# liudabao001/JABD-Joint-Attention-Based-Detector-for-small-face-detection

Hardware: AMD Instinct MI355X
Metric: images/sec at 1024x1024 bs32 (1/2/4/8 GPU); boxes/sec NMS (higher is better)
Workload: dtype fp32; 1 GPU; C2: JABD-MobileNetV3 RetinaFace (nets/retinaface_r.py) eval forward, weights_init weights; global_batch=32, image_size=1024, parallelism=replicas x1

## Files before the change

jabd-joint-attention-based-detector-for-small-face-detection_amd/csrc/expdw.hip:

```cpp
#include "expdw_shared.h"

namespace jabd {

template <int K, int S, int TH, int TW, int EC, bool SKIP, int NW, int SKC>
constexpr int xd1_min_wg() {
  using C = XdCfg<K, S, TH, TW, EC>;
  constexpr int bytes = C::LDS * 4 + K * K * (EC / 4) * 16 + (SKIP ? 10 * (SKC / 4) * 16 : 16);
  return (SKIP && NW == 4 && 4 * bytes <= 160 * 1024) ? 4 : 2;
}

template <int K, int S, int TH, int TW, int EC, int ACT, int KP, bool SKIP = false, int NW = 4,
          int SKC = 160, int KCC = 0, bool PRE = false>
__global__ __launch_bounds__(64 * NW, (xd1_min_wg<K, S, TH, TW, EC, SKIP, NW, SKC>())) void expdw1_kernel(const jabd_expdw_args p, const XdDivs dv,
                                                       int nitems) {
  static_assert(!PRE || (KCC == 1 && KP == 1), "PRE: one input stage");
  const int Kc = KCC ? KCC : p.Kc;
  using C = XdCfg<K, S, TH, TW, EC>;
  constexpr int T = 64 * NW;
  constexpr int NPF = (C::IPAD * 4 + T - 1) / T;
  constexpr int BPW = (C::NBLK + NW - 1) / NW;
  static_assert(NW % C::NNT == 0, "waves split evenly over the 16-channel tiles");
  constexpr int NWD = K * K * C::NC4;
  __shared__ __attribute__((aligned(16))) float lds[C::LDS];
  __shared__ float4 wsh[K * K][C::NC4];
  __shared__ float4 sws[SKIP ? 10 : 1][SKIP ? SKC / 4 : 1];
  XdItem it;
  XD_RT(0);
  XD_T(1);
  if (!xd_item<K, S, TH, TW, EC>(p, blockIdx.x, dv, nitems, it)) return;
  const bool skip = SKIP && it.c0 == 0;
  if (skip) {
    const int c4 = threadIdx.x & 63;
    if (c4 < (p.Cin >> 2))
      for (int q = threadIdx.x >> 6; q < 10; q += NW)
        sws[q][c4] = *reinterpret_cast<const float4*>((q < 9 ? p.sw + q * p.Cin : p.sb) + 4 * c4);
  }
  const bool interior =
      it.ih0 >= 0 && it.iw0 >= 0 && it.ih0 + C::IH <= p.H && it.iw0 + C::IW <= p.W;
  const int t = threadIdx.x, lane = t & 63, wave = t >> 6, j = lane & 15, g = lane >> 4;
  const int ntw = wave % C::NNT;
  const int nt = it.c0 / 16 + ntw;
  const bool ntv = nt < p.Ntiles;
  const int ntc = ntv ? nt : 0;
  const f32x4* wpk = reinterpret_cast<const f32x4*>(p.we);
  const int chb = it.c0 + 16 * ntw + 4 * g;
  const bool chok = chb < p.E;
  float4 pbi = *reinterpret_cast<const float4*>(p.be + (chok ? chb : 0));
  if (!chok) pbi = make_float4(0.f, 0.f, 0.f, 0.f);
  float4 pwd = make_float4(0.f, 0.f, 0.f, 0.f);
  if (t < NWD) {
    const int tp = t / C::NC4, cc = it.c0 + 4 * (t - tp * C::NC4);
    const float4 w = *reinterpret_cast<const float4*>(p.wd + tp * p.E + (cc < p.E ? cc : 0));
    pwd = cc < p.E ? w : make_float4(0.f, 0.f, 0.f, 0.f);
  }
  int c4, sl;
  dw_lane<C::NC4>(lane, c4, sl);
  const int chl = 4 * c4;
  const bool chv = it.c0 + chl < p.E;
  const float4 bias2 = *reinterpret_cast<const float4*>(p.bd + (chv ? it.c0 + chl : 0));
  f32x4 apre = (f32x4){0.f, 0.f, 0.f, 0.f};
  float4 bpre = make_float4(0.f, 0.f, 0.f, 0.f);
  if constexpr (PRE) {
    const f32x4 w = reinterpret_cast<const f32x4*>(p.pw)[lane];
    const float4 gt = *reinterpret_cast<const float4*>(p.pg + (int64_t)it.b * p.pg_bs + 4 * g);
    apre = (f32x4){w.x * gt.x, w.y * gt.y, w.z * gt.z, w.w * gt.w};
    bpre = *reinterpret_cast<const float4*>(p.pb + 4 * g);
  }
  const __amdgpu_buffer_rsrc_t xr = __builtin_amdgcn_make_buffer_rsrc(
      const_cast<float*>(p.x), (short)0, (int)(uint32_t)((int64_t)p.B * p.x_bs * 4), 0x00020000);
  const int cq = ((t >> 4) & 3) * 4;
  const int spx0 = (t >> 6) * 16 + (t & 15);
  float4 pf[KP][NPF];
  auto load_stage = [&](int kc, float4 (&dst)[NPF]) {
    const int cofs = 16 * kc + cq;
    const uint32_t base = (uint32_t)(it.b * p.x_bs + cofs);
    const bool cok = cofs < p.Cin;
#pragma unroll
    for (int u = 0; u < NPF; ++u) {
      const int px = u * 16 * NW + spx0;
      const int r = px / C::IW, c = px - r * C::IW;
      const int ih = it.ih0 + r, iw = it.iw0 + c;
      const bool ok = px < C::IPX && cok &&
                      (interior || ((unsigned)ih < (unsigned)p.H && (unsigned)iw < (unsigned)p.W));
      const uint32_t off = ok ? (base + (uint32_t)((ih * p.W + iw) * p.x_ps)) * 4u : 0xFFFFFFF0u;
      if (XD_SKIP & 16) dst[u] = make_float4(0.f, 0.f, 0.f, (float)off);
      else dst[u] = __builtin_bit_cast(float4, __builtin_amdgcn_raw_buffer_load_b128(xr, off, 0, 0));
    }
  };
  f32x4 acc[BPW];
  const f32x4 bias4 = (f32x4){pbi.x, pbi.y, pbi.z, pbi.w};
#pragma unroll
  for (int u = 0; u < BPW; ++u) acc[u] = bias4;
#pragma unroll
  for (int s = 0; s < KP; ++s)
    if (s < Kc) load_stage(s, pf[s]);
  const bool tail8 = KCC == 2 && (p.Cin & 15) == 8;
  for (int kc0 = 0; kc0 < Kc; kc0 += KP) {
#pragma unroll
    for (int s = 0; s < KP; ++s) {
      const int kc = kc0 + s;
      if (kc >= Kc) break;
      const bool tl = tail8 && kc == Kc - 1;
      f32x4 a;
      if (tl) {
        const float* wf = reinterpret_cast<const float*>(p.we) +
                          ((int64_t)(kc * p.Ntiles + ntc) * 64 + j) * 4 + g;
        a = (f32x4){wf[0], wf[64], 0.f, 0.f};
      } else {
        a = wpk[(kc * p.Ntiles + ntc) * 64 + lane];
      }
#pragma unroll
      for (int u = 0; u < NPF; ++u) {
        if (u * 16 * NW + spx0 < C::IPAD)
          *reinterpret_cast<float4*>(lds + (cq / 4 * C::IPAD + u * 16 * NW + spx0) * 4) = pf[s][u];
      }
      if (!ntv) a = (f32x4){0.f, 0.f, 0.f, 0.f};
      asm volatile("" : "+v"(a));
      lds_barrier();
      if (kc == 0) XD_T(2);
      if constexpr (PRE) {
        constexpr int BPP = (C::NPB + NW - 1) / NW;
        const __amdgpu_buffer_rsrc_t rr = __builtin_amdgcn_make_buffer_rsrc(
            const_cast<float*>(p.pres), (short)0, (int)(uint32_t)((int64_t)p.B * p.x_bs * 4),
            0x00020000);
        f32x4 pacc[BPP];
        float4 res[BPP];
        bool pin[BPP];
#pragma unroll
        for (int u = 0; u < BPP; ++u) {
          const int pb = wave + NW * u;
          const int px = pb * 16 + j;
          const int r = px / C::IW, c = px - r * C::IW;
          const int ih = it.ih0 + r, iw = it.iw0 + c;
          pin[u] = pb < C::NPB && px < C::IPX &&
                   (interior || ((unsigned)ih < (unsigned)p.H && (unsigned)iw < (unsigned)p.W));
          const uint32_t off =
              pin[u] ? (uint32_t)(it.b * p.x_bs + (ih * p.W + iw) * p.x_ps + 4 * g) * 4u : 0xFFFFFFF0u;
          res[u] = __builtin_bit_cast(float4, __builtin_amdgcn_raw_buffer_load_b128(rr, off, 0, 0));
          pacc[u] = (f32x4){bpre.x, bpre.y, bpre.z, bpre.w};
          if (pb < C::NPB) {
            const f32x4 bv = *reinterpret_cast<const f32x4*>(lds + (g * C::IPAD + px) * 4);
            pacc[u] = __builtin_amdgcn_mfma_f32_16x16x4f32(apre.x, bv.x, pacc[u], 0, 0, 0);
            pacc[u] = __builtin_amdgcn_mfma_f32_16x16x4f32(apre.y, bv.y, pacc[u], 0, 0, 0);
            pacc[u] = __builtin_amdgcn_mfma_f32_16x16x4f32(apre.z, bv.z, pacc[u], 0, 0, 0);
            pacc[u] = __builtin_amdgcn_mfma_f32_16x16x4f32(apre.w, bv.w, pacc[u], 0, 0, 0);
          }
        }
        lds_barrier();
#pragma unroll
        for (int u = 0; u < BPP; ++u) {
          const int pb = wave + NW * u;
          if (pb >= C::NPB) continue;
          float4 v = make_float4(pacc[u][0] + res[u].x, pacc[u][1] + res[u].y,
                                 pacc[u][2] + res[u].z, pacc[u][3] + res[u].w);
          if (p.pact == ACT_RELU) v = xd_act4<ACT_RELU>(v);
          else if (p.pact == ACT_HSWISH) v = xd_act4<ACT_HSWISH>(v);
          if (!pin[u]) v = make_float4(0.f, 0.f, 0.f, 0.f);
          *reinterpret_cast<float4*>(lds + (g * C::IPAD + pb * 16 + j) * 4) = v;
        }
        lds_barrier();
      }
      if (kc + KP < Kc) load_stage(kc + KP, pf[s]);
      const int sc = 16 * kc + 4 * (t >> 6);
      if (skip && wave < 4 && sc < p.Cin) {
        const int op = t & 63, orow = op / TW, ocol = op - orow * TW;
        const int oh = it.oh0 + orow, ow = it.ow0 + ocol;
        if (orow < TH && oh < p.OH && ow < p.OW) {
          const int sq = sc >> 2;
          float4 v = sws[9][sq];
          const float* xq = lds + ((t >> 6) * C::IPAD) * 4;
#pragma unroll 1
          for (int kh = 0; kh < 3; ++kh)
#pragma unroll
            for (int kw = 0; kw < 3; ++kw) {
              const int px = (2 * orow + kh + C::PAD - 1) * C::IW + 2 * ocol + kw + C::PAD - 1;
              const float4 xv = *reinterpret_cast<const float4*>(xq + px * 4);
              const float4 wv = sws[kh * 3 + kw][sq];
              v = fma4pk(xv, wv, v);
            }
          *reinterpret_cast<float4*>(p.sy + (int64_t)it.b * p.sy_bs +
                                     ((int64_t)oh * p.OW + ow) * p.sy_ps + sc) = v;
        }
      }
      if (ntv && !(XD_SKIP & 1) && tl) {
#pragma unroll
        for (int u = 0; u < BPW; ++u) {
          const int blk = wave + NW * u;
          if (blk < C::NBLK) {
            const int pb = blk / C::NNT;
            const float b0 = lds[(pb * 16 + j) * 4 + g];
            const float b1 = lds[(C::IPAD + pb * 16 + j) * 4 + g];
            acc[u] = __builtin_amdgcn_mfma_f32_16x16x4f32(a.x, b0, acc[u], 0, 0, 0);
            acc[u] = __builtin_amdgcn_mfma_f32_16x16x4f32(a.y, b1, acc[u], 0, 0, 0);
          }
        }
      } else if (ntv && !(XD_SKIP & 1)) {
#pragma unroll
        for (int u = 0; u < BPW; ++u) {
          const int blk = wave + NW * u;
          if (blk < C::NBLK) {
            const int pb = blk / C::NNT;
            const f32x4 bv = *reinterpret_cast<const f32x4*>(lds + (g * C::IPAD + pb * 16 + j) * 4);
            acc[u] = __builtin_amdgcn_mfma_f32_16x16x4f32(a.x, bv.x, acc[u], 0, 0, 0);
            acc[u] = __builtin_amdgcn_mfma_f32_16x16x4f32(a.y, bv.y, acc[u], 0, 0, 0);
            acc[u] = __builtin_amdgcn_mfma_f32_16x16x4f32(a.z, bv.z, acc[u], 0, 0, 0);
            acc[u] = __builtin_amdgcn_mfma_f32_16x16x4f32(a.w, bv.w, acc[u], 0, 0, 0);
          }
        }
      }
      lds_barrier();
    }
  }
  XD_T(3);
  if (XD_SKIP & 2) {
  } else if (interior) {
#pragma unroll
    for (int u = 0; u < BPW; ++u) {
      const int blk = wave + NW * u;
      if (blk < C::NBLK) {
        const int pb = blk / C::NNT;
        const int px = pb * 16 + j, q = 4 * ntw + g;
        const float4 o = xd_act4<ACT>(make_float4(acc[u][0], acc[u][1], acc[u][2], acc[u][3]));
        if (pb * 16 + 16 <= C::IPX || px < C::IPX)
          *reinterpret_cast<float4*>(lds + (q * C::QP + px) * 4) = o;
      }
    }
  } else {
#pragma unroll
    for (int u = 0; u < BPW; ++u) {
      const int blk = wave + NW * u;
      if (blk < C::NBLK) {
        const int pb = blk / C::NNT;
        const int px = pb * 16 + j, q = 4 * ntw + g;
        const int r = px / C::IW, c = px - r * C::IW;
        const int ih = it.ih0 + r, iw = it.iw0 + c;
        const bool ok = (unsigned)ih < (unsigned)p.H && (unsigned)iw < (unsigned)p.W;
        float4 o = xd_act4<ACT>(make_float4(acc[u][0], acc[u][1], acc[u][2], acc[u][3]));
        if (!ok) o = make_float4(0.f, 0.f, 0.f, 0.f);
        if (px < C::IPX) *reinterpret_cast<float4*>(lds + (q * C::QP + px) * 4) = o;
      }
    }
  }
  if (t < NWD) wsh[t / C::NC4][t % C::NC4] = pwd;
  __syncthreads();
  XD_T(4);

  constexpr int SPW = 64 / C::NC4;
  float4 psum = make_float4(0.f, 0.f, 0.f, 0.f);
  if (chv && !(XD_SKIP & 4)) {
    float* yb = p.y + (int64_t)it.b * p.y_bs + it.c0 + chl;
#pragma unroll 1
    for (int pass = 0; pass * T < C::ITEMS; ++pass) {
      const int strip = (pass * NW + wave) * SPW + sl;
      if (strip >= TH * C::NSTRIP) break;
      const int orow = strip / C::NSTRIP, st = strip - orow * C::NSTRIP;
      const int oh = it.oh0 + orow, owb = it.ow0 + st * C::PW;
      if (oh >= p.OH || owb >= p.OW) continue;
      float4 a2[C::PW];
#pragma unroll
      for (int o = 0; o < C::PW; ++o) a2[o] = bias2;
#pragma unroll 1
      for (int kh = 0; kh < K; ++kh) {
        const float* rowp = lds + (c4 * C::QP + (orow * S + kh) * C::IW + st * C::PW * S) * 4;
        float4 row[C::SPAN];
#pragma unroll
        for (int c = 0; c < C::SPAN; ++c)
          row[c] = *reinterpret_cast<const float4*>(rowp + c * 4);
        float4 wk[K];
#pragma unroll
        for (int kw = 0; kw < K; ++kw) wk[kw] = wsh[kh * K + kw][c4];
#pragma unroll
        for (int o = 0; o < C::PW; ++o)
#pragma unroll
          for (int kw = 0; kw < K; ++kw) {
            const float4 xv = row[o * S + kw], wv = wk[kw];
            a2[o] = fma4pk(xv, wv, a2[o]);
          }
      }
#pragma unroll
      for (int o = 0; o < C::PW; ++o) {
        if (owb + o >= p.OW) break;
        const float4 v = xd_act4<ACT>(a2[o]);
        *reinterpret_cast<float4*>(yb + ((int64_t)oh * p.OW + owb + o) * p.y_ps) = v;
        psum.x += v.x; psum.y += v.y; psum.z += v.z; psum.w += v.w;
      }
    }
  }
  XD_T(5);
  if (p.part && !(XD_SKIP & 8)) {
    constexpr int NX = C::NC4 == 16 ? 2 : C::NC4 == 8 ? 3 : 4;
    constexpr int X8[3] = {12, 20, 32}, X4[4] = {4, 8, 16, 32}, X16[2] = {16, 32};
#pragma unroll
    for (int r = 0; r < NX; ++r) {
      const int off = C::NC4 == 16 ? X16[r] : C::NC4 == 8 ? X8[r] : X4[r];
      psum.x += __shfl_xor(psum.x, off);
      psum.y += __shfl_xor(psum.y, off);
      psum.z += __shfl_xor(psum.z, off);
      psum.w += __shfl_xor(psum.w, off);
    }
    __syncthreads();
    float4* red = reinterpret_cast<float4*>(lds);
    if (lane < C::NC4) red[wave * C::NC4 + lane] = psum;
    __syncthreads();
    if (t < C::NC4 && it.c0 + 4 * t < p.E) {
      float4 v[NW];
#pragma unroll
      for (int w = 0; w < NW; ++w) v[w] = red[w * C::NC4 + t];
#pragma unroll
      for (int h = NW / 2; h >= 1; h >>= 1)
#pragma unroll
        for (int w = 0; w < h; ++w) {
          v[w].x += v[w + h].x;
          v[w].y += v[w + h].y;
          v[w].z += v[w + h].z;
          v[w].w += v[w + h].w;
        }
      const float4 sm = v[0];
      *reinterpret_cast<float4*>(p.part + ((int64_t)it.b * (int)dv.tiles_img.d + it.t_in) * p.E +
                                 it.c0 + 4 * t) = sm;
    }
  }
  XD_T(6);
  XD_RT(7);
}


template <int K, int EC, int NB, int R>
struct XsCfg {
  static constexpr int PAD = K / 2;
  static constexpr int NPX = 16 * NB, OWS = NPX - 2 * PAD;
  static constexpr int NR = R + 2 * PAD;
  static constexpr int EP = EC + 4;
  static constexpr int NT = EC / 16, NC4 = EC / 4;
  static constexpr int SPX = R * NPX;
  static constexpr int NPF = SPX * 4 / 256;
  static constexpr int NBLK = R * NB * NT, BPW = NBLK / 4;
  static constexpr int PW = 2, NSTRIP = OWS / PW;
  static constexpr int ITEMS = R * NSTRIP * NC4;
  static constexpr int SPAN = PW + K - 1;
  static constexpr int LDS_X = 16 * SPX, LDS_E = NR * NPX * EP;
  static_assert(SPX * 4 % 256 == 0 && NBLK % 4 == 0 && 4 % NT == 0, "strip shape");
  static_assert(OWS % PW == 0, "strip width");
  static_assert((LDS_X + LDS_E) * 4 + (K * K + 1) * EC * 4 <= 80 * 1024, "LDS");
  static_assert(LDS_X >= 4 * 256, "ECA reduction buffer aliases the stage buffer");
};

template <int K, int EC, int NB, int R, int ACT>
__global__ __launch_bounds__(256, 2) void expdw_strip_kernel(const jabd_expdw_args p,
                                                             const XdDivs dv, int nitems,
                                                             int nstrip, int hb) {
  using C = XsCfg<K, EC, NB, R>;
  __shared__ __attribute__((aligned(16))) float xs[C::LDS_X];
  __shared__ __attribute__((aligned(16))) float er[C::LDS_E];
  __shared__ float4 wsh[K * K + 1][C::NC4];
  float4* red = reinterpret_cast<float4*>(xs);
  const int i = blockIdx.x;
  if (i >= nitems) return;
  const int xcd = i & 7, q = i >> 3;
  const int qn = fdiv(q, dv.nch);
  const int chunk = q - qn * (int)dv.nch.d;
  const int tile = qn * 8 + xcd;
  if (tile >= p.B * (int)dv.tiles_img.d) return;
  const int b = fdiv(tile, dv.tiles_img);
  const int t_in = tile - b * (int)dv.tiles_img.d;
  const int band = t_in / nstrip, strip = t_in - band * nstrip;
  const int hb0 = band * hb, hb1 = min(hb0 + hb, p.OH);
  const int ow0 = strip * C::OWS, iw0 = ow0 - C::PAD;
  const int c0 = chunk * EC;
  const int t = threadIdx.x, lane = t & 63, j = lane & 15, g = lane >> 4;
  const int wave = t >> 6;
  const int ntw = wave % C::NT;
  const int nt = c0 / 16 + ntw;
  const bool ntv = nt < p.Ntiles;
  const int ntc = ntv ? nt : 0;
  const f32x4* wpk = reinterpret_cast<const f32x4*>(p.we);
  const int chb = c0 + 16 * ntw + 4 * g;
  const bool chok = chb < p.E;
  const float4 pbi = *reinterpret_cast<const float4*>(p.be + (chok ? chb : 0));
  const f32x4 bias4 = (f32x4){pbi.x, pbi.y, pbi.z, pbi.w};
  for (int u = t; u < (K * K + 1) * C::NC4; u += 256) {
    const int tp = u / C::NC4, cc = c0 + 4 * (u - tp * C::NC4);
    const float4 w = *reinterpret_cast<const float4*>((tp < K * K ? p.wd + tp * p.E : p.bd) +
                                                      (cc < p.E ? cc : 0));
    wsh[tp][u - tp * C::NC4] = cc < p.E ? w : make_float4(0.f, 0.f, 0.f, 0.f);
  }
  const __amdgpu_buffer_rsrc_t xr = __builtin_amdgcn_make_buffer_rsrc(
      const_cast<float*>(p.x), (short)0, (int)(uint32_t)((int64_t)p.B * p.x_bs * 4), 0x00020000);
  const int cq = ((t >> 4) & 3) * 4;
  const int spx0 = (t >> 6) * 16 + (t & 15);
  const int e0 = hb0 - C::PAD;
  const int nsteps = (hb1 - hb0 + 2 * C::PAD + R - 1) / R;
  const int nitem = nsteps * p.Kc;
  float4 pf[C::NPF];
  auto load_stage = [&](int it) {
    const int s = it / p.Kc, kc = it - s * p.Kc;
    const int cofs = 16 * kc + cq;
    const uint32_t base = (uint32_t)(b * p.x_bs + cofs);
    const bool cok = cofs < p.Cin;
#pragma unroll
    for (int u = 0; u < C::NPF; ++u) {
      const int px = u * 64 + spx0;
      const int r = px / C::NPX, c = px - r * C::NPX;
      const int ih = e0 + s * R + r, iw = iw0 + c;
      const bool ok = cok && (unsigned)ih < (unsigned)p.H && (unsigned)iw < (unsigned)p.W;
      const uint32_t off = ok ? (base + (uint32_t)((ih * p.W + iw) * p.x_ps)) * 4u : 0xFFFFFFF0u;
      pf[u] = __builtin_bit_cast(float4, __builtin_amdgcn_raw_buffer_load_b128(xr, off, 0, 0));
    }
  };
  int c4, sl;
  dw_lane<C::NC4>(lane, c4, sl);
  const int chl = 4 * c4;
  const bool chv = c0 + chl < p.E;
  float* yb = p.y + (int64_t)b * p.y_bs + c0 + chl;
  float4 psum = make_float4(0.f, 0.f, 0.f, 0.f);
  f32x4 acc[C::BPW];
  load_stage(0);
  for (int it = 0; it < nitem; ++it) {
    const int s = it / p.Kc, kc = it - s * p.Kc;
    if (kc == 0) {
#pragma unroll
      for (int u = 0; u < C::BPW; ++u) acc[u] = bias4;
    }
    f32x4 a = wpk[(kc * p.Ntiles + ntc) * 64 + lane];
#pragma unroll
    for (int u = 0; u < C::NPF; ++u)
      *reinterpret_cast<float4*>(xs + ((cq / 4) * C::SPX + u * 64 + spx0) * 4) = pf[u];
    if (!ntv) a = (f32x4){0.f, 0.f, 0.f, 0.f};
    asm volatile("" : "+v"(a));
    lds_barrier();
    if (it + 1 < nitem) load_stage(it + 1);
    if (ntv) {
#pragma unroll
      for (int u = 0; u < C::BPW; ++u) {
        const int pb = (wave + 4 * u) / C::NT;
        const f32x4 bv = *reinterpret_cast<const f32x4*>(xs + (g * C::SPX + pb * 16 + j) * 4);
        acc[u] = __builtin_amdgcn_mfma_f32_16x16x4f32(a.x, bv.x, acc[u], 0, 0, 0);
        acc[u] = __builtin_amdgcn_mfma_f32_16x16x4f32(a.y, bv.y, acc[u], 0, 0, 0);
        acc[u] = __builtin_amdgcn_mfma_f32_16x16x4f32(a.z, bv.z, acc[u], 0, 0, 0);
        acc[u] = __builtin_amdgcn_mfma_f32_16x16x4f32(a.w, bv.w, acc[u], 0, 0, 0);
      }
    }
    if (kc + 1 < p.Kc) {
      lds_barrier();
      continue;
    }
#pragma unroll
    for (int u = 0; u < C::BPW; ++u) {
      const int pb = (wave + 4 * u) / C::NT;
      const int px = pb * 16 + j;
      const int r = px / C::NPX, c = px - r * C::NPX;
      const int ih = e0 + s * R + r, iw = iw0 + c;
      const bool ok = chok && (unsigned)ih < (unsigned)p.H && (unsigned)iw < (unsigned)p.W;
      const int slot = (s * R + r) % C::NR;
      float4 o;
      o.x = ok ? xd_act<ACT>(acc[u][0]) : 0.f;
      o.y = ok ? xd_act<ACT>(acc[u][1]) : 0.f;
      o.z = ok ? xd_act<ACT>(acc[u][2]) : 0.f;
      o.w = ok ? xd_act<ACT>(acc[u][3]) : 0.f;
      *reinterpret_cast<float4*>(er + (slot * C::NPX + c) * C::EP + 16 * ntw + 4 * g) = o;
    }
    lds_barrier();
    if (chv) {
      const float4 bias2 = wsh[K * K][c4];
#pragma unroll 1
      for (int pass = 0; pass * 256 < C::ITEMS; ++pass) {
        const int item = (pass * 4 + wave) * (64 / C::NC4) + sl;
        if (item >= R * C::NSTRIP) break;
        const int orow = item / C::NSTRIP, st = item - orow * C::NSTRIP;
        const int oh = hb0 + s * R - 2 * C::PAD + orow;
        const int owb = ow0 + st * C::PW;
        if (oh < hb0 || oh >= hb1 || owb >= p.OW) continue;
        float4 a2[C::PW];
#pragma unroll
        for (int o = 0; o < C::PW; ++o) a2[o] = bias2;
#pragma unroll 1
        for (int kh = 0; kh < K; ++kh) {
          const int slot = (oh - e0 - C::PAD + kh) % C::NR;
          const float* rowp = er + (slot * C::NPX + st * C::PW) * C::EP + chl;
          float4 row[C::SPAN];
#pragma unroll
          for (int c = 0; c < C::SPAN; ++c)
            row[c] = *reinterpret_cast<const float4*>(rowp + c * C::EP);
          float4 wk[K];
#pragma unroll
          for (int kw = 0; kw < K; ++kw) wk[kw] = wsh[kh * K + kw][c4];
#pragma unroll
          for (int o = 0; o < C::PW; ++o)
#pragma unroll
            for (int kw = 0; kw < K; ++kw) {
              const float4 xv = row[o + kw], wv = wk[kw];
              a2[o] = fma4pk(xv, wv, a2[o]);
            }
        }
#pragma unroll
        for (int o = 0; o < C::PW; ++o) {
          if (owb + o >= p.OW) break;
          float4 v;
          v.x = xd_act<ACT>(a2[o].x);
          v.y = xd_act<ACT>(a2[o].y);
          v.z = xd_act<ACT>(a2[o].z);
          v.w = xd_act<ACT>(a2[o].w);
          *reinterpret_cast<float4*>(yb + ((int64_t)oh * p.OW + owb + o) * p.y_ps) = v;
          psum.x += v.x; psum.y += v.y; psum.z += v.z; psum.w += v.w;
        }
      }
    }
    lds_barrier();
  }
  if (p.part) {
    __syncthreads();
    red[t] = psum;
    __syncthreads();
    if (t < C::NC4 && c0 + 4 * t < p.E) {
      float4 sm = make_float4(0.f, 0.f, 0.f, 0.f);
      for (int u = 0; u < 256; ++u) {
        int cu, su;
        dw_lane<C::NC4>(u & 63, cu, su);
        if (cu != t) continue;
        const float4 v = red[u];
        sm.x += v.x; sm.y += v.y; sm.z += v.z; sm.w += v.w;
      }
      *reinterpret_cast<float4*>(p.part + ((int64_t)b * (int)dv.tiles_img.d + t_in) * p.E + c0 +
                                 4 * t) = sm;
    }
  }
}

#ifndef XW_NE
#define XW_NE 4
#endif
template <int K, int S, int TH, int TW, int EC, bool SKIP>
struct XwCfg {
  using C = XdCfg<K, S, TH, TW, EC>;
  static constexpr int NE = XW_NE, NT = 64 * (NE + 4);
  static constexpr int NBW = (C::NPB + NE - 1) / NE;
  static constexpr int SKC = SKIP ? 160 : 4;
  static constexpr int OFF_W = 2 * C::LDS_E * 4;
  static constexpr int OFF_R = OFF_W + 2 * (K * K + 1) * C::NC4 * 16;
  static constexpr int OFF_S = OFF_R + 2 * 4 * C::NC4 * 16;
  static constexpr int BYTES = OFF_S + 10 * (SKC / 4) * 16;
  static_assert(BYTES <= 160 * 1024, "LDS");
};

template <int NBW, int NNT>
struct XwSlot {
  float4 b[NBW];
  f32x4 a[NNT];
  float4 bias[NNT];
  float4 taps;
};

template <int NBW, int NNT>
__device__ __forceinline__ void xw_touch(XwSlot<NBW, NNT>& sl) {
#pragma unroll
  for (int u = 0; u < NBW; ++u)
    asm volatile("" : "+v"(sl.b[u].x), "+v"(sl.b[u].y), "+v"(sl.b[u].z), "+v"(sl.b[u].w));
#pragma unroll
  for (int nt = 0; nt < NNT; ++nt) {
    asm volatile("" : "+v"(sl.a[nt]));
    asm volatile("" : "+v"(sl.bias[nt].x), "+v"(sl.bias[nt].y), "+v"(sl.bias[nt].z),
                 "+v"(sl.bias[nt].w));
  }
  asm volatile("" : "+v"(sl.taps.x), "+v"(sl.taps.y), "+v"(sl.taps.z), "+v"(sl.taps.w));
}

template <int NBU, int NTU, int NBW, int NNT>
__device__ __forceinline__ void xw_mfma(f32x4 (&acc)[NBW][NNT], const XwSlot<NBW, NNT>& sl) {
#pragma unroll
  for (int e = 0; e < 4; ++e)
#pragma unroll
    for (int u = 0; u < NBU; ++u)
#pragma unroll
      for (int nt = 0; nt < NTU; ++nt) {
        const float av = e == 0 ? sl.a[nt].x : e == 1 ? sl.a[nt].y : e == 2 ? sl.a[nt].z : sl.a[nt].w;
        const float bv = e == 0 ? sl.b[u].x : e == 1 ? sl.b[u].y : e == 2 ? sl.b[u].z : sl.b[u].w;
        acc[u][nt] = __builtin_amdgcn_mfma_f32_16x16x4f32(av, bv, acc[u][nt], 0, 0, 0);
      }
}

template <int K, int S, int TH, int TW, int EC, int ACT, bool SKIP, int D>
__global__ __launch_bounds__(64 * (XW_NE + 4)) void expdw_ws_kernel(const jabd_expdw_args p, const XdDivs dv,
                                                      int nitems) {
  using C = XdCfg<K, S, TH, TW, EC>;
  using W = XwCfg<K, S, TH, TW, EC, SKIP>;
  constexpr int NBW = W::NBW, NNT = C::NNT, NC4 = C::NC4, NE = W::NE;
  constexpr int NWD = (K * K + 1) * NC4;
  static_assert(NWD <= 64 * NE, "taps: one float4 per expand thread");
  extern __shared__ __attribute__((aligned(16))) unsigned char xw_smem[];
  float* ebuf = reinterpret_cast<float*>(xw_smem);
// ... 165 lines not shown
  const int chl = 4 * c4;
  constexpr int SPW = 64 / NC4;
  lds_barrier();
  for (int n = 0; n < nmine; ++n) {
    XdItem it;
    const bool valid = decode(n, it);
    if (valid && SKIP && it.c0 == 0) {
      const int nq = p.Cin >> 2;
      for (int i = dt; i < 64 * nq; i += 256) {
        const int sq = i >> 6, op = i & 63, orow = op / TW, ocol = op - orow * TW;
        const int oh = it.oh0 + orow, ow = it.ow0 + ocol;
        if (orow >= TH || oh >= p.OH || ow >= p.OW) continue;
        float4 v = sws[9 * (W::SKC / 4) + sq];
        const uint32_t base = (uint32_t)(it.b * p.x_bs + 4 * sq);
#pragma unroll 1
        for (int kh = 0; kh < 3; ++kh)
#pragma unroll
          for (int kw = 0; kw < 3; ++kw) {
            const int ih = 2 * oh + kh - 1, iw = 2 * ow + kw - 1;
            const bool ok = (unsigned)ih < (unsigned)p.H && (unsigned)iw < (unsigned)p.W;
            const uint32_t off = ok ? (base + (uint32_t)((ih * p.W + iw) * p.x_ps)) * 4u : 0xFFFFFFF0u;
            const float4 xv =
                __builtin_bit_cast(float4, __builtin_amdgcn_raw_buffer_load_b128(xr, off, 0, 0));
            const float4 wv = sws[(kh * 3 + kw) * (W::SKC / 4) + sq];
            v = fma4pk(xv, wv, v);
          }
        *reinterpret_cast<float4*>(p.sy + (int64_t)it.b * p.sy_bs +
                                   ((int64_t)oh * p.OW + ow) * p.sy_ps + 4 * sq) = v;
      }
    }
    float4 psum = make_float4(0.f, 0.f, 0.f, 0.f);
    if (valid && it.c0 + chl < p.E && !(XD_SKIP & 64)) {
      const float* eb = ebuf + (n & 1) * C::LDS_E;
      const float4* wb = wsh + (n & 1) * (K * K + 1) * NC4;
      const float4 bias2 = wb[K * K * NC4 + c4];
      float* yb = p.y + (int64_t)it.b * p.y_bs + it.c0 + chl;
#pragma unroll 1
      for (int pass = 0; pass * 256 < C::ITEMS; ++pass) {
        const int strip = (pass * 4 + dwv) * SPW + sl;
        if (strip >= TH * C::NSTRIP) break;
        const int orow = strip / C::NSTRIP, st = strip - orow * C::NSTRIP;
        const int oh = it.oh0 + orow, owb = it.ow0 + st * C::PW;
        if (oh >= p.OH || owb >= p.OW) continue;
        float4 a2[C::PW];
#pragma unroll
        for (int o = 0; o < C::PW; ++o) a2[o] = bias2;
#pragma unroll 1
        for (int kh = 0; kh < K; ++kh) {
          const float* rowp = eb + ((orow * S + kh) * C::IW + st * C::PW * S) * C::EP + chl;
          float4 row[C::SPAN];
#pragma unroll
          for (int c = 0; c < C::SPAN; ++c)
            row[c] = *reinterpret_cast<const float4*>(rowp + c * C::EP);
          float4 wk[K];
#pragma unroll
          for (int kw = 0; kw < K; ++kw) wk[kw] = wb[(kh * K + kw) * NC4 + c4];
#pragma unroll
          for (int o = 0; o < C::PW; ++o)
#pragma unroll
            for (int kw = 0; kw < K; ++kw) {
              const float4 xv = row[o * S + kw], wv = wk[kw];
              a2[o] = fma4pk(xv, wv, a2[o]);
            }
        }
#pragma unroll
        for (int o = 0; o < C::PW; ++o) {
          if (owb + o >= p.OW) break;
          float4 v;
          v.x = xd_act<ACT>(a2[o].x);
          v.y = xd_act<ACT>(a2[o].y);
          v.z = xd_act<ACT>(a2[o].z);
          v.w = xd_act<ACT>(a2[o].w);
          *reinterpret_cast<float4*>(yb + ((int64_t)oh * p.OW + owb + o) * p.y_ps) = v;
          psum.x += v.x; psum.y += v.y; psum.z += v.z; psum.w += v.w;
        }
      }
    }
    if (p.part) {
      constexpr int NX = NC4 == 8 ? 3 : 4;
      constexpr int X8[3] = {12, 20, 32}, X4[4] = {4, 8, 16, 32};
#pragma unroll
      for (int r = 0; r < NX; ++r) {
        const int off = NC4 == 8 ? X8[r] : X4[r];
        psum.x += __shfl_xor(psum.x, off);
        psum.y += __shfl_xor(psum.y, off);
        psum.z += __shfl_xor(psum.z, off);
        psum.w += __shfl_xor(psum.w, off);
      }
      if (lane < NC4) red[(n & 1) * 4 * NC4 + dwv * NC4 + lane] = psum;
      if (n >= 1) finalize(n - 1);
    }
    lds_barrier();
  }
  if (p.part && nmine >= 1) finalize(nmine - 1);
}

#ifndef XW_D
#define XW_D 2
#endif

XdTile xd_tile(int k, int s) {
  if (s == 1) return k == 3 ? XdTile{14, 16} : XdTile{16, 16};
  return XdTile{8, 8};
}

int xd_skc(int cin) { return cin <= 40 ? 40 : cin <= 112 ? 112 : 160; }

}

using namespace jabd;

static int xd_kp() {
  static int kp = -1;
  if (kp < 0) {
    const char* e = getenv("JABD_EXPDW_KP");
    kp = e && (e[0] == '2' || e[0] == '3') ? e[0] - '0' : 1;
  }
  return kp;
}

static int xd_nw(const jabd_expdw_args& a, int EC) {
  static int env = -1;
  if (env < 0) {
    const char* e = getenv("JABD_EXPDW_NW");
    env = e && e[0] == '8' ? 8 : (e && e[0] == '4' ? 4 : 0);
  }
  (void)a;
  (void)EC;
  if (env) return env;
  return 4;
}

static bool xs_enabled() {
  static int on = -1;
  if (on < 0) {
    const char* e = getenv("JABD_EXPDW_STRIP");
    on = e && e[0] == '1' ? 1 : 0;
  }
  return on == 1;
}

static int xw_form = 0;
static bool xw_enabled() {
  static int env = -1;
  if (env < 0) {
    const char* e = getenv("JABD_EXPDW_WS");
    env = e && e[0] == '1' ? 1 : 0;
  }
  return xw_form ? xw_form == 2 : env == 1;
}
static bool x2_enabled() {
  static int env = -1;
  if (env < 0) {
    const char* e = getenv("JABD_EXPDW2");
    env = e && e[0] == '1' ? 1 : 0;
  }
  return xw_form ? xw_form == 3 : env == 1;
}

template <int K, int S, int TH, int TW, int EC, int ACT, bool SKIP>
static int xw_launch(const jabd_expdw_args& a, const XdDivs& dv, int64_t nitems, hipStream_t st) {
  constexpr int D = XW_D;
  auto kern = expdw_ws_kernel<K, S, TH, TW, EC, ACT, SKIP, D>;
  constexpr int bytes = XwCfg<K, S, TH, TW, EC, SKIP>::BYTES;
  static int occ = -1, ncu = 0;
  if (occ < 0) {
    int dev = 0;
    JABD_HIP(hipGetDevice(&dev));
    JABD_HIP(hipDeviceGetAttribute(&ncu, hipDeviceAttributeMultiprocessorCount, dev));
    JABD_HIP(hipFuncSetAttribute((const void*)kern, hipFuncAttributeMaxDynamicSharedMemorySize, bytes));
    int o = 0;
    JABD_HIP(hipOccupancyMaxActiveBlocksPerMultiprocessor(&o, kern, XwCfg<K, S, TH, TW, EC, SKIP>::NT,
                                                          bytes));
    occ = o < 1 ? 1 : o;
  }
  JABD_REQUIRE((int64_t)a.B * a.x_bs * 4 <= 0xFFFFF000ll - 1024,
               "expand_dw: input must be < 4 GiB - 5 KiB (split the batch)");
  const int64_t cap = (int64_t)ncu * occ;
  const int grid = (int)(nitems < cap ? nitems : cap);
  kern<<<grid, XwCfg<K, S, TH, TW, EC, SKIP>::NT, bytes, st>>>(a, dv, (int)nitems);
  return check_launch("expand_dw_ws");
}

struct XsPlan {
  int nb, nstrip, hb, nband;
};

static XsPlan xs_plan(int OH, int OW, int k) {
  XsPlan pl;
  int best = 0;
  for (int nb = 2; nb <= 3; ++nb) {
    const int ows = 16 * nb - 2 * (k / 2);
    const int ns = (int)cdiv(OW, ows);
    if (!best || ns * 16 * nb < best) {
      best = ns * 16 * nb;
      pl.nb = nb;
      pl.nstrip = ns;
    }
  }
  pl.hb = OH >= 256 ? 64 : 32;
  pl.nband = (int)cdiv(OH, pl.hb);
  return pl;
}

#if XD_TRACE
extern "C" int jabd_xd_trace_set(void* buf) {
  unsigned long long* p = static_cast<unsigned long long*>(buf);
  JABD_HIP(hipMemcpyToSymbol(HIP_SYMBOL(xd_trace_buf), &p, sizeof(p)));
  return JABD_OK;
}
#endif

extern "C" int jabd_expand_dw_select(int32_t form) {
  const int prev = xw_form;
  xw_form = form >= 1 && form <= 4 ? form : 0;
  return prev;
}

extern "C" int64_t jabd_expand_dw_nblk(int32_t OH, int32_t OW, int32_t k, int32_t stride) {
  if (OH <= 0 || OW <= 0 || (stride != 1 && stride != 2)) return -1;
  if (stride == 1 && xs_enabled()) {
    const XsPlan pl = xs_plan(OH, OW, k);
    return (int64_t)pl.nband * pl.nstrip;
  }
  const XdTile tl = xd_tile(k, stride);
  return cdiv(OH, tl.th) * cdiv(OW, tl.tw);
}

extern "C" int jabd_expand_dw_nhwc_f32(const jabd_expdw_args* args, jabd_stream_t stream) {
  JABD_REQUIRE(args, "expand_dw: null args");
  const jabd_expdw_args& a = *args;
  JABD_REQUIRE(a.x && a.we && a.be && a.wd && a.bd && a.y, "expand_dw: null pointer");
  JABD_REQUIRE(a.Cin % 4 == 0 && a.x_ps % 4 == 0 && a.E % 4 == 0 && a.y_ps % 4 == 0 &&
                   a.y_ps >= a.E && a.x_ps >= a.Cin,
               "expand_dw: channel counts / strides must be multiples of 4");
  JABD_REQUIRE(a.Kc == (a.Cin + 15) / 16 && a.Ntiles * 16 >= a.E, "expand_dw: packing mismatch");
  JABD_REQUIRE((a.k == 3 || a.k == 5) && (a.stride == 1 || a.stride == 2) &&
                   a.OH == (a.H + 2 * (a.k / 2) - a.k) / a.stride + 1 &&
                   a.OW == (a.W + 2 * (a.k / 2) - a.k) / a.stride + 1,
               "expand_dw: unsupported geometry");
  JABD_REQUIRE(a.act == ACT_NONE || a.act == ACT_RELU || a.act == ACT_HSWISH,
               "expand_dw: act %d", a.act);
  JABD_REQUIRE(!a.sy || (a.stride == 2 && a.sw && a.sb && a.sy_ps % 4 == 0 && a.sy_ps >= a.Cin &&
                         a.Cin <= 160),
               "expand_dw: the fused skip branch needs stride 2, Cin <= 160, weights, bias and "
               "sy_ps %% 4 == 0");
  if (a.stride == 1 && xs_enabled()) {
    const XsPlan pl = xs_plan(a.OH, a.OW, a.k);
    const int tiles_img = pl.nband * pl.nstrip;
    JABD_REQUIRE(!a.part || a.nblk == tiles_img, "expand_dw: nblk %d != %d", a.nblk, tiles_img);
    const int EC = a.E <= 16 ? 16 : 32;
    const int nch = (int)cdiv(a.E, EC);
    const int64_t nitems = cdiv((int64_t)a.B * tiles_img, 8) * 8 * nch;
    JABD_REQUIRE(nitems < ((int64_t)1 << 31) && (int64_t)a.H * a.W * a.x_ps < ((int64_t)1 << 31) &&
                     (int64_t)a.B * a.x_bs * 4 < ((int64_t)1 << 32) - 16,
                 "expand_dw: problem too large for 32-bit indexing / buffer offsets (split the batch)");
    const XdDivs dv{make_fastdiv((uint32_t)nch), make_fastdiv((uint32_t)tiles_img),
                    make_fastdiv((uint32_t)pl.nstrip)};
    hipStream_t st = as_stream(stream);
#define XS_LAUNCH(K_, EC_, NB_, ACT_)                                                       \
  expdw_strip_kernel<K_, EC_, NB_, 4, ACT_><<<(unsigned)nitems, 256, 0, st>>>(a, dv, (int)nitems, \
                                                                             pl.nstrip, pl.hb)
#define XS_ACTS(K_, EC_, NB_)                              \
  if (a.k == K_ && EC == EC_ && pl.nb == NB_) {            \
    if (a.act == ACT_RELU)                                 \
      XS_LAUNCH(K_, EC_, NB_, ACT_RELU);                   \
    else if (a.act == ACT_HSWISH)                          \
      XS_LAUNCH(K_, EC_, NB_, ACT_HSWISH);                 \
    else                                                   \
      XS_LAUNCH(K_, EC_, NB_, ACT_NONE);                   \
    return check_launch("expand_dw_strip");                \
  }
    XS_ACTS(3, 16, 2) XS_ACTS(3, 16, 3) XS_ACTS(3, 32, 2) XS_ACTS(3, 32, 3)
    XS_ACTS(5, 16, 2) XS_ACTS(5, 16, 3) XS_ACTS(5, 32, 2) XS_ACTS(5, 32, 3)
#undef XS_ACTS
#undef XS_LAUNCH
    set_error("expand_dw: no strip kernel for k=%d", a.k);
    return JABD_EINVAL;
  }
  const XdTile tl = xd_tile(a.k, a.stride);
  const int tiles_w = (int)cdiv(a.OW, tl.tw);
  const int tiles_img = (int)cdiv(a.OH, tl.th) * tiles_w;
  JABD_REQUIRE(!a.part || a.nblk == tiles_img, "expand_dw: nblk %d != %d", a.nblk, tiles_img);
  static int ec16 = -1;
  if (ec16 < 0) {
    const char* e = getenv("JABD_EXPDW_EC16");
    ec16 = e && e[0] == '1' ? 1 : 0;
  }
  const int EC = (a.E <= 16 || ec16 || (a.k == 5 && a.stride == 2 && a.Cin <= 32)) ? 16 : 32;
  const int nch = (int)cdiv(a.E, EC);
  const int64_t ntiles = (int64_t)a.B * tiles_img;
  const int64_t nitems = cdiv(ntiles, 8) * 8 * nch;
  JABD_REQUIRE(nitems < ((int64_t)1 << 31) && (int64_t)a.H * a.W * a.x_ps < ((int64_t)1 << 31),
               "expand_dw: problem too large for 32-bit item / pixel indexing");
  JABD_REQUIRE((int64_t)a.B * a.x_bs * 4 < ((int64_t)1 << 32),
               "expand_dw: input must be < 4 GiB (split the batch)");
  const int nw = xd_nw(a, EC);
  const int skc = xd_skc(a.Cin);
  hipStream_t st = as_stream(stream);
  const XdDivs dv{make_fastdiv((uint32_t)nch), make_fastdiv((uint32_t)tiles_img),
                  make_fastdiv((uint32_t)tiles_w)};
  JABD_REQUIRE((int64_t)a.B * a.x_bs * 4 < ((int64_t)1 << 32) - 16,
               "expand_dw: input must be < 4 GiB (buffer-descriptor offsets)");
  if (a.pw) {
    JABD_REQUIRE(a.pb && a.pg && a.pres && a.pg_bs >= a.Cin &&
                     (a.pact == ACT_NONE || a.pact == ACT_RELU || a.pact == ACT_HSWISH),
                 "expand_dw: bad fused-project arguments");
    JABD_REQUIRE(a.k == 3 && a.stride == 2 && EC == 32 && a.sy && a.Cin == 16 && a.Kc == 1 &&
                     a.x_ps == 16 && skc == 40 && nw == 4,
                 "expand_dw: the fused previous project takes the 3x3/s2 Cin-16 skip form only");
    static int pre_ec = -1;
    if (pre_ec < 0) {
      const char* e = getenv("JABD_EXPDW_PRE_EC");
      pre_ec = e && e[0] == '3' ? 32 : 64;
    }
    if (pre_ec == 64 && a.E <= 64) {
      const XdDivs dv1{make_fastdiv(1u), dv.tiles_img, dv.tiles_w};
      const int64_t n1 = cdiv(ntiles, 8) * 8;
#define XP_LAUNCH(ACT_)                                                                        \
  expdw1_kernel<3, 2, 8, 8, 64, ACT_, 1, true, 8, 40, 1, true><<<(unsigned)n1, 512, 0, st>>>( \
      a, dv1, (int)n1)
      if (a.act == ACT_RELU)
        XP_LAUNCH(ACT_RELU);
      else if (a.act == ACT_HSWISH)
        XP_LAUNCH(ACT_HSWISH);
      else
        XP_LAUNCH(ACT_NONE);
#undef XP_LAUNCH
      return check_launch("expand_dw (fused project, one chunk)");
    }
#define XP_LAUNCH(ACT_)                                                                       \
  expdw1_kernel<3, 2, 8, 8, 32, ACT_, 1, true, 4, 40, 1, true><<<(unsigned)nitems, 256, 0, st>>>( \
      a, dv, (int)nitems)
    if (a.act == ACT_RELU)
      XP_LAUNCH(ACT_RELU);
    else if (a.act == ACT_HSWISH)
      XP_LAUNCH(ACT_HSWISH);
    else
      XP_LAUNCH(ACT_NONE);
#undef XP_LAUNCH
    return check_launch("expand_dw (fused project)");
  }
  if (xw_form == 0 || xw_form == 4) {
    const int e = expdw3_dispatch(a, dv, tiles_img, xw_form == 4, st);
    if (e != JABD_EINVAL) return e;
  }
  if (x2_enabled() && !xw_enabled()) {
    const int e = expdw2_dispatch(a, dv, nitems, EC, nch, st);
    if (e != JABD_EINVAL) return e;
  }
  if (xw_enabled()) {
#define XW_ACT(K_, S_, TH_, TW_, EC_, SK_)                                         \
  {                                                                              \
    if (a.act == ACT_RELU) return xw_launch<K_, S_, TH_, TW_, EC_, ACT_RELU, SK_>(a, dv, nitems, st);     \
    if (a.act == ACT_HSWISH) return xw_launch<K_, S_, TH_, TW_, EC_, ACT_HSWISH, SK_>(a, dv, nitems, st); \
    return xw_launch<K_, S_, TH_, TW_, EC_, ACT_NONE, SK_>(a, dv, nitems, st);                           \
  }
#define XW_CASE(K_, S_, TH_, TW_, EC_)                          \
  if (a.k == K_ && a.stride == S_ && EC == EC_) {               \
    if (S_ == 2 && a.sy) XW_ACT(K_, S_, TH_, TW_, EC_, true)    \
    XW_ACT(K_, S_, TH_, TW_, EC_, false)                        \
  }
    XW_CASE(3, 1, 14, 16, 16) XW_CASE(3, 1, 14, 16, 32)
    XW_CASE(5, 1, 16, 16, 16) XW_CASE(5, 1, 16, 16, 32)
    XW_CASE(3, 2, 8, 8, 16) XW_CASE(3, 2, 8, 8, 32)
    XW_CASE(5, 2, 8, 8, 16) XW_CASE(5, 2, 8, 8, 32)
#undef XW_CASE
#undef XW_ACT
  }
#define XD_LAUNCH(K_, S_, TH_, TW_, EC_, ACT_)                                                \
  do {                                                                                        \
    if (S_ == 2 && a.sy && nw == 8)                                                           \
      expdw1_kernel<K_, S_, TH_, TW_, EC_, ACT_, 1, true, 8><<<(unsigned)nitems, 512, 0, st>>>( \
          a, dv, (int)nitems);                                                                \
    else if (S_ == 2 && a.sy && skc == 40 && a.Kc == 2)                                       \
      expdw1_kernel<K_, S_, TH_, TW_, EC_, ACT_, 1, true, 4, 40, 2><<<(unsigned)nitems, 256, 0, st>>>( \
          a, dv, (int)nitems);                                                                \
    else if (S_ == 2 && a.sy && skc == 40)                                                    \
      expdw1_kernel<K_, S_, TH_, TW_, EC_, ACT_, 1, true, 4, 40><<<(unsigned)nitems, 256, 0, st>>>( \
          a, dv, (int)nitems);                                                                \
    else if (S_ == 2 && a.sy && skc == 112)                                                   \
      expdw1_kernel<K_, S_, TH_, TW_, EC_, ACT_, 1, true, 4, 112><<<(unsigned)nitems, 256, 0, st>>>( \
          a, dv, (int)nitems);                                                                \
    else if (S_ == 2 && a.sy)                                                                 \
      expdw1_kernel<K_, S_, TH_, TW_, EC_, ACT_, 1, true><<<(unsigned)nitems, 256, 0, st>>>( \
          a, dv, (int)nitems);                                                                \
    else if (nw == 8)                                                                         \
      expdw1_kernel<K_, S_, TH_, TW_, EC_, ACT_, 1, false, 8><<<(unsigned)nitems, 512, 0, st>>>( \
          a, dv, (int)nitems);                                                                \
    else if (a.Kc == 1)                                                                       \
      expdw1_kernel<K_, S_, TH_, TW_, EC_, ACT_, 1, false, 4, 160, 1><<<(unsigned)nitems, 256, 0, st>>>( \
          a, dv, (int)nitems);                                                                \
    else if (a.Kc == 2)                                                                       \
      expdw1_kernel<K_, S_, TH_, TW_, EC_, ACT_, 2, false, 4, 160, 2><<<(unsigned)nitems, 256, 0, st>>>( \
          a, dv, (int)nitems);                                                                \
    else if (xd_kp() == 1)                                                                    \
      expdw1_kernel<K_, S_, TH_, TW_, EC_, ACT_, 1><<<(unsigned)nitems, 256, 0, st>>>(       \
          a, dv, (int)nitems);                                                                \
    else if (xd_kp() == 2)                                                                    \
      expdw1_kernel<K_, S_, TH_, TW_, EC_, ACT_, 2><<<(unsigned)nitems, 256, 0, st>>>(       \
          a, dv, (int)nitems);                                                                \
    else                                                                                      \
      expdw1_kernel<K_, S_, TH_, TW_, EC_, ACT_, 3><<<(unsigned)nitems, 256, 0, st>>>(       \
          a, dv, (int)nitems);                                                                \
  } while (0)
#define XD_CASE(K_, S_, TH_, TW_, EC_)                                    \
  if (a.k == K_ && a.stride == S_ && EC == EC_) {                         \
    if (a.act == ACT_RELU)                                                \
      XD_LAUNCH(K_, S_, TH_, TW_, EC_, ACT_RELU);                         \
    else if (a.act == ACT_HSWISH)                                         \
      XD_LAUNCH(K_, S_, TH_, TW_, EC_, ACT_HSWISH);                       \
    else                                                                  \
      XD_LAUNCH(K_, S_, TH_, TW_, EC_, ACT_NONE);                         \
    return check_launch("expand_dw");                                     \
  }
  XD_CASE(3, 1, 14, 16, 16) XD_CASE(3, 1, 14, 16, 32)
  XD_CASE(5, 1, 16, 16, 16) XD_CASE(5, 1, 16, 16, 32)
  XD_CASE(3, 2, 8, 8, 16) XD_CASE(3, 2, 8, 8, 32)
  XD_CASE(5, 2, 8, 8, 16) XD_CASE(5, 2, 8, 8, 32)
#undef XD_CASE
#undef XD_LAUNCH
  set_error("expand_dw: no kernel for k=%d stride=%d", a.k, a.stride);
  return JABD_EINVAL;
}
```

Before: 4991 images/sec.

## Precompute input offsets, hoist residual loads, use buffer stores in expand-depthwise kernel

Input load offsets are now computed once per pixel slot and reused across channel stages by adding a per-stage stride. In the fused-project path the residual loads are issued before the barrier, and one LDS barrier is removed. The depthwise bias is staged through shared memory instead of a global load. The output loop is restructured with row-pointer increments and a compile-time full-tile variant that drops bounds checks, and output stores go through buffer descriptors. This cuts integer address math and barrier stalls, but adds an LDS row and relies on the barrier removal and the new offset reuse being correct.

```diff
diff --git a/jabd-joint-attention-based-detector-for-small-face-detection_amd/csrc/expdw.hip b/jabd-joint-attention-based-detector-for-small-face-detection_amd/csrc/expdw.hip
--- a/jabd-joint-attention-based-detector-for-small-face-detection_amd/csrc/expdw.hip
+++ b/jabd-joint-attention-based-detector-for-small-face-detection_amd/csrc/expdw.hip
@@ -1,3 +1,5 @@
+#include <type_traits>
+
 #include "expdw_shared.h"
 
 namespace jabd {
@@ -5,7 +7,7 @@
 template <int K, int S, int TH, int TW, int EC, bool SKIP, int NW, int SKC>
 constexpr int xd1_min_wg() {
   using C = XdCfg<K, S, TH, TW, EC>;
-  constexpr int bytes = C::LDS * 4 + K * K * (EC / 4) * 16 + (SKIP ? 10 * (SKC / 4) * 16 : 16);
+  constexpr int bytes = C::LDS * 4 + (K * K + 1) * (EC / 4) * 16 + (SKIP ? 10 * (SKC / 4) * 16 : 16);
   return (SKIP && NW == 4 && 4 * bytes <= 160 * 1024) ? 4 : 2;
 }
 
@@ -20,9 +22,9 @@
   constexpr int NPF = (C::IPAD * 4 + T - 1) / T;
   constexpr int BPW = (C::NBLK + NW - 1) / NW;
   static_assert(NW % C::NNT == 0, "waves split evenly over the 16-channel tiles");
-  constexpr int NWD = K * K * C::NC4;
+  constexpr int NWD = (K * K + 1) * C::NC4;
   __shared__ __attribute__((aligned(16))) float lds[C::LDS];
-  __shared__ float4 wsh[K * K][C::NC4];
+  __shared__ float4 wsh[K * K + 1][C::NC4];
   __shared__ float4 sws[SKIP ? 10 : 1][SKIP ? SKC / 4 : 1];
   XdItem it;
   XD_RT(0);
@@ -50,14 +52,14 @@
   float4 pwd = make_float4(0.f, 0.f, 0.f, 0.f);
   if (t < NWD) {
     const int tp = t / C::NC4, cc = it.c0 + 4 * (t - tp * C::NC4);
-    const float4 w = *reinterpret_cast<const float4*>(p.wd + tp * p.E + (cc < p.E ? cc : 0));
+    const float4 w = *reinterpret_cast<const float4*>((tp < K * K ? p.wd + tp * p.E : p.bd) +
+                                                      (cc < p.E ? cc : 0));
     pwd = cc < p.E ? w : make_float4(0.f, 0.f, 0.f, 0.f);
   }
   int c4, sl;
   dw_lane<C::NC4>(lane, c4, sl);
   const int chl = 4 * c4;
   const bool chv = it.c0 + chl < p.E;
-  const float4 bias2 = *reinterpret_cast<const float4*>(p.bd + (chv ? it.c0 + chl : 0));
   f32x4 apre = (f32x4){0.f, 0.f, 0.f, 0.f};
   float4 bpre = make_float4(0.f, 0.f, 0.f, 0.f);
   if constexpr (PRE) {
@@ -70,23 +72,32 @@
       const_cast<float*>(p.x), (short)0, (int)(uint32_t)((int64_t)p.B * p.x_bs * 4), 0x00020000);
   const int cq = ((t >> 4) & 3) * 4;
   const int spx0 = (t >> 6) * 16 + (t & 15);
-  float4 pf[KP][NPF];
-  auto load_stage = [&](int kc, float4 (&dst)[NPF]) {
-    const int cofs = 16 * kc + cq;
-    const uint32_t base = (uint32_t)(it.b * p.x_bs + cofs);
-    const bool cok = cofs < p.Cin;
+  constexpr uint32_t XD_OOR = 0xFFFFFFF0u;
+  uint32_t soff[NPF];
+  {
+    const uint32_t base = (uint32_t)(it.b * p.x_bs + cq);
 #pragma unroll
     for (int u = 0; u < NPF; ++u) {
       const int px = u * 16 * NW + spx0;
       const int r = px / C::IW, c = px - r * C::IW;
       const int ih = it.ih0 + r, iw = it.iw0 + c;
-      const bool ok = px < C::IPX && cok &&
+      const bool ok = px < C::IPX &&
                       (interior || ((unsigned)ih < (unsigned)p.H && (unsigned)iw < (unsigned)p.W));
-      const uint32_t off = ok ? (base + (uint32_t)((ih * p.W + iw) * p.x_ps)) * 4u : 0xFFFFFFF0u;
+      soff[u] = ok ? (base + (uint32_t)((ih * p.W + iw) * p.x_ps)) * 4u : XD_OOR;
+    }
+  }
+  float4 pf[KP][NPF];
+  auto load_stage = [&](int kc, float4 (&dst)[NPF]) {
+    const bool cok = 16 * kc + cq < p.Cin;
+#pragma unroll
+    for (int u = 0; u < NPF; ++u) {
+      const bool ok = (int)cok & (int)(soff[u] != XD_OOR);
+      const uint32_t off = ok ? soff[u] + 64u * (uint32_t)kc : XD_OOR;
       if (XD_SKIP & 16) dst[u] = make_float4(0.f, 0.f, 0.f, (float)off);
       else dst[u] = __builtin_bit_cast(float4, __builtin_amdgcn_raw_buffer_load_b128(xr, off, 0, 0));
     }
   };
+  typedef decltype(__builtin_amdgcn_raw_buffer_load_b128(xr, 0u, 0, 0)) b128_t;
   f32x4 acc[BPW];
   const f32x4 bias4 = (f32x4){pbi.x, pbi.y, pbi.z, pbi.w};
 #pragma unroll
@@ -95,6 +106,9 @@
   for (int s = 0; s < KP; ++s)
     if (s < Kc) load_stage(s, pf[s]);
   const bool tail8 = KCC == 2 && (p.Cin & 15) == 8;
+  constexpr int BPP = (C::NPB + NW - 1) / NW;
+  static_assert(!PRE || BPP == NPF, "PRE: one stage slot per project block");
+  float4 res[PRE ? BPP : 1];
   for (int kc0 = 0; kc0 < Kc; kc0 += KP) {
 #pragma unroll
     for (int s = 0; s < KP; ++s) {
@@ -109,6 +123,14 @@
       } else {
         a = wpk[(kc * p.Ntiles + ntc) * 64 + lane];
       }
+      if constexpr (PRE) {
+        const __amdgpu_buffer_rsrc_t rr = __builtin_amdgcn_make_buffer_rsrc(
+            const_cast<float*>(p.pres), (short)0, (int)(uint32_t)((int64_t)p.B * p.x_bs * 4),
+            0x00020000);
+#pragma unroll
+        for (int u = 0; u < BPP; ++u)
+          res[u] = __builtin_bit_cast(float4, __builtin_amdgcn_raw_buffer_load_b128(rr, soff[u], 0, 0));
+      }
 #pragma unroll
       for (int u = 0; u < NPF; ++u) {
         if (u * 16 * NW + spx0 < C::IPAD)
@@ -119,24 +141,11 @@
       lds_barrier();
       if (kc == 0) XD_T(2);
       if constexpr (PRE) {
-        constexpr int BPP = (C::NPB + NW - 1) / NW;
-        const __amdgpu_buffer_rsrc_t rr = __builtin_amdgcn_make_buffer_rsrc(
-            const_cast<float*>(p.pres), (short)0, (int)(uint32_t)((int64_t)p.B * p.x_bs * 4),
-            0x00020000);
         f32x4 pacc[BPP];
-        float4 res[BPP];
-        bool pin[BPP];
 #pragma unroll
         for (int u = 0; u < BPP; ++u) {
           const int pb = wave + NW * u;
           const int px = pb * 16 + j;
-          const int r = px / C::IW, c = px - r * C::IW;
-          const int ih = it.ih0 + r, iw = it.iw0 + c;
-          pin[u] = pb < C::NPB && px < C::IPX &&
-                   (interior || ((unsigned)ih < (unsigned)p.H && (unsigned)iw < (unsigned)p.W));
-          const uint32_t off =
-              pin[u] ? (uint32_t)(it.b * p.x_bs + (ih * p.W + iw) * p.x_ps + 4 * g) * 4u : 0xFFFFFFF0u;
-          res[u] = __builtin_bit_cast(float4, __builtin_amdgcn_raw_buffer_load_b128(rr, off, 0, 0));
           pacc[u] = (f32x4){bpre.x, bpre.y, bpre.z, bpre.w};
           if (pb < C::NPB) {
             const f32x4 bv = *reinterpret_cast<const f32x4*>(lds + (g * C::IPAD + px) * 4);
@@ -146,7 +155,6 @@
             pacc[u] = __builtin_amdgcn_mfma_f32_16x16x4f32(apre.w, bv.w, pacc[u], 0, 0, 0);
           }
         }
-        lds_barrier();
 #pragma unroll
         for (int u = 0; u < BPP; ++u) {
           const int pb = wave + NW * u;
@@ -155,7 +163,7 @@
                                  pacc[u][2] + res[u].z, pacc[u][3] + res[u].w);
           if (p.pact == ACT_RELU) v = xd_act4<ACT_RELU>(v);
           else if (p.pact == ACT_HSWISH) v = xd_act4<ACT_HSWISH>(v);
-          if (!pin[u]) v = make_float4(0.f, 0.f, 0.f, 0.f);
+          if (soff[u] == XD_OOR) v = make_float4(0.f, 0.f, 0.f, 0.f);
           *reinterpret_cast<float4*>(lds + (g * C::IPAD + pb * 16 + j) * 4) = v;
         }
         lds_barrier();
@@ -178,8 +186,13 @@
               const float4 wv = sws[kh * 3 + kw][sq];
               v = fma4pk(xv, wv, v);
             }
-          *reinterpret_cast<float4*>(p.sy + (int64_t)it.b * p.sy_bs +
-                                     ((int64_t)oh * p.OW + ow) * p.sy_ps + sc) = v;
+          const __amdgpu_buffer_rsrc_t sr = __builtin_amdgcn_make_buffer_rsrc(
+              p.sy + (int64_t)it.b * p.sy_bs, (short)0,
+              (int)(((uint32_t)(p.OH * p.OW - 1) * (uint32_t)p.sy_ps + (uint32_t)p.Cin) * 4u),
+              0x00020000);
+          __builtin_amdgcn_raw_buffer_store_b128(
+              __builtin_bit_cast(b128_t, v), sr,
+              (uint32_t)((oh * p.OW + ow) * p.sy_ps + sc) * 4u, 0, 0);
         }
       }
       if (ntv && !(XD_SKIP & 1) && tl) {
@@ -248,43 +261,60 @@
   constexpr int SPW = 64 / C::NC4;
   float4 psum = make_float4(0.f, 0.f, 0.f, 0.f);
   if (chv && !(XD_SKIP & 4)) {
-    float* yb = p.y + (int64_t)it.b * p.y_bs + it.c0 + chl;
+    const __amdgpu_buffer_rsrc_t yr = __builtin_amdgcn_make_buffer_rsrc(
+        p.y + (int64_t)it.b * p.y_bs, (short)0,
+        (int)(((uint32_t)(p.OH * p.OW - 1) * (uint32_t)p.y_ps + (uint32_t)p.E) * 4u), 0x00020000);
+    const float4 bias2 = wsh[K * K][c4];
+    static_assert((NW * SPW) % C::NSTRIP == 0, "a pass covers whole tile rows");
+    constexpr int RPP = NW * SPW / C::NSTRIP;
+    const int strip0 = wave * SPW + sl;
+    const int orow0 = strip0 / C::NSTRIP, st = strip0 - orow0 * C::NSTRIP;
+    const int owb = it.ow0 + st * C::PW;
+    const float* rowp0 = lds + (c4 * C::QP + orow0 * S * C::IW + st * C::PW * S) * 4;
+    const uint32_t ystep = (uint32_t)p.y_ps * 4u;
+    const uint32_t yoff0 = ((uint32_t)((it.oh0 + orow0) * p.OW + owb) * (uint32_t)p.y_ps +
+                            (uint32_t)(it.c0 + chl)) * 4u;
+    auto dw_phase = [&](auto fullc) {
+      constexpr bool FULL = decltype(fullc)::value;
+      const float* rowq = rowp0;
+      uint32_t yoff = yoff0;
 #pragma unroll 1
-    for (int pass = 0; pass * T < C::ITEMS; ++pass) {
-      const int strip = (pass * NW + wave) * SPW + sl;
-      if (strip >= TH * C::NSTRIP) break;
-      const int orow = strip / C::NSTRIP, st = strip - orow * C::NSTRIP;
-      const int oh = it.oh0 + orow, owb = it.ow0 + st * C::PW;
-      if (oh >= p.OH || owb >= p.OW) continue;
-      float4 a2[C::PW];
-#pragma unroll
-      for (int o = 0; o < C::PW; ++o) a2[o] = bias2;
+      for (int orow = orow0; orow < TH;
+           orow += RPP, rowq += RPP * S * C::IW * 4, yoff += (uint32_t)RPP * p.OW * ystep) {
+        if (!FULL && (it.oh0 + orow >= p.OH || owb >= p.OW)) continue;
+        float4 a2[C::PW];
+#pragma unroll
+        for (int o = 0; o < C::PW; ++o) a2[o] = bias2;
 #pragma unroll 1
-      for (int kh = 0; kh < K; ++kh) {
-        const float* rowp = lds + (c4 * C::QP + (orow * S + kh) * C::IW + st * C::PW * S) * 4;
-        float4 row[C::SPAN];
-#pragma unroll
-        for (int c = 0; c < C::SPAN; ++c)
-          row[c] = *reinterpret_cast<const float4*>(rowp + c * 4);
-        float4 wk[K];
-#pragma unroll
-        for (int kw = 0; kw < K; ++kw) wk[kw] = wsh[kh * K + kw][c4];
-#pragma unroll
-        for (int o = 0; o < C::PW; ++o)
-#pragma unroll
-          for (int kw = 0; kw < K; ++kw) {
-            const float4 xv = row[o * S + kw], wv = wk[kw];
-            a2[o] = fma4pk(xv, wv, a2[o]);
-          }
-      }
-#pragma unroll
-      for (int o = 0; o < C::PW; ++o) {
-        if (owb + o >= p.OW) break;
-        const float4 v = xd_act4<ACT>(a2[o]);
-        *reinterpret_cast<float4*>(yb + ((int64_t)oh * p.OW + owb + o) * p.y_ps) = v;
-        psum.x += v.x; psum.y += v.y; psum.z += v.z; psum.w += v.w;
-      }
-    }
+        for (int kh = 0; kh < K; ++kh) {
+          const float* rowp = rowq + kh * C::IW * 4;
+          float4 row[C::SPAN];
+#pragma unroll
+          for (int c = 0; c < C::SPAN; ++c)
+            row[c] = *reinterpret_cast<const float4*>(rowp + c * 4);
+          float4 wk[K];
+#pragma unroll
+          for (int kw = 0; kw < K; ++kw) wk[kw] = wsh[kh * K + kw][c4];
+#pragma unroll
+          for (int o = 0; o < C::PW; ++o)
+#pragma unroll
+            for (int kw = 0; kw < K; ++kw) {
+              const float4 xv = row[o * S + kw], wv = wk[kw];
+              a2[o] = fma4pk(xv, wv, a2[o]);
+            }
+        }
+#pragma unroll
+        for (int o = 0; o < C::PW; ++o) {
+          if (!FULL && owb + o >= p.OW) break;
+          const float4 v = xd_act4<ACT>(a2[o]);
+          __builtin_amdgcn_raw_buffer_store_b128(__builtin_bit_cast(b128_t, v), yr,
+                                                 yoff + (uint32_t)o * ystep, 0, 0);
+          psum.x += v.x; psum.y += v.y; psum.z += v.z; psum.w += v.w;
+        }
+      }
+    };
+    if (it.oh0 + TH <= p.OH && it.ow0 + TW <= p.OW) dw_phase(std::true_type{});
+    else dw_phase(std::false_type{});
   }
   XD_T(5);
   if (p.part && !(XD_SKIP & 8)) {
@@ -1056,6 +1086,9 @@
                   make_fastdiv((uint32_t)tiles_w)};
   JABD_REQUIRE((int64_t)a.B * a.x_bs * 4 < ((int64_t)1 << 32) - 16,
                "expand_dw: input must be < 4 GiB (buffer-descriptor offsets)");
+  JABD_REQUIRE((int64_t)a.OH * a.OW * a.y_ps * 4 < ((int64_t)1 << 32) &&
+                   (!a.sy || (int64_t)a.OH * a.OW * a.sy_ps * 4 < ((int64_t)1 << 32)),
+               "expand_dw: one image of the output must be < 4 GiB");
   if (a.pw) {
     JABD_REQUIRE(a.pb && a.pg && a.pres && a.pg_bs >= a.Cin &&
                      (a.pact == ACT_NONE || a.pact == ACT_RELU || a.pact == ACT_HSWISH),
```

Result: faster. 5079 images/sec, median of 6 (+1.8%).
